# yui-mhcp/text_to_speech

Measured on AMD Instinct MI355X. Metric: audio samples/sec (22.05 kHz WaveGlow vocoding, fp32), higher is better.
Workload: dtype f32; 1 GPU; WaveGlow-only vocoding of precomputed 80x800 mel, batch 8 per GPU, fp32 (BASELINE.json configs[1]); batch_per_gpu=8, mel_frames=800, world_size=1, backend=single process, weights=seeded synthetic (rng 1234)

## Files before the change

### text_to_speech_amd/csrc/engine.h

```cpp
#pragma once
#include <hip/hip_runtime.h>
#include <stdint.h>

#include <cstdio>
#include <functional>
#include <map>
#include <string>
#include <tuple>
#include <vector>

#include "../../include/tts_hip.h"

#include "ttsw_host.h"
#include "wg_call.h"

struct DevBuf {
    void* p = nullptr;
    size_t bytes = 0;
    hipError_t ensure(size_t need) {
        if (need <= bytes) return hipSuccess;
        if (p) (void)hipFree(p);
        p = nullptr;
        bytes = 0;
        hipError_t e = hipMalloc(&p, need);
// ... 178 lines not shown
    std::map<std::string, HostTensor> host;
    WaveGlowDev wg;
    Tacotron2Dev taco;
    MelStftDev stft;
    AudioProcDev aproc;
    ResampleDev resamp;
    bool timing = false;
    std::vector<TimedLaunch> timed;
    std::vector<TimedLaunch> ev_pool;
    double time_sum_us[4] = {0, 0, 0, 0};
    int64_t time_cnt[4] = {0, 0, 0, 0};
};

int set_err(const tts_hip_engine* e, int code, const char* fmt, ...);

struct StreamScope {
    tts_hip_engine* e;
    hipStream_t saved;
    StreamScope(tts_hip_engine* eng, void* stream) : e(eng), saved(eng->stream) {
        if (stream) e->stream = (hipStream_t)stream;
    }
    ~StreamScope() { e->stream = saved; }
};

#define HIPCHK(e, call)                                                                                         \
    do {                                                                                                        \
        hipError_t _err = (call);                                                                               \
        if (_err != hipSuccess)                                                                                 \
            return set_err((e), TTS_HIP_EHIP, "%s:%d: %s -> %s", __FILE__, __LINE__, #call, hipGetErrorString(_err)); \
    } while (0)

int waveglow_build_wino(tts_hip_engine* e);
int waveglow_wino_begin(tts_hip_engine* e, const float* d_mel, int PR, int BT, int T, int form);
int waveglow_wino_layer(tts_hip_engine* e, const WgLayerDev& ly, int i, const float* x, float* acts_i, int PR, int BT, int T);
int waveglow_wino_layer0(tts_hip_engine* e, const WgLayerDev& ly, int h, const float* a0p, float* acts_0, int PR, int BT, int T);
void timing_begin(tts_hip_engine* e, int kind);
void timing_end(tts_hip_engine* e);
void timing_collect(tts_hip_engine* e);

int waveglow_finalize(tts_hip_engine* e);
int waveglow_run(tts_hip_engine* e, const float* d_mel, int B, int T, const float* d_z, float sigma, float* d_audio,
                 int precision, const int* d_lens = nullptr, const int* d_tail = nullptr, int n_tail = 0,
                 const int* d_flags = nullptr);
int waveglow_run_packed(tts_hip_engine* e, const float* d_mel, int B, int T, const float* d_z, float sigma, float* d_audio,
                        int precision, const int* d_info, int F, int n_gap);
void waveglow_free(tts_hip_engine* e);

int tacotron2_finalize(tts_hip_engine* e);
void tacotron2_free(tts_hip_engine* e);

int melstft_finalize(tts_hip_engine* e);
int melstft_run(tts_hip_engine* e, const float* d_audio, int B, int N, float* d_mel);
void melstft_free(tts_hip_engine* e);
void audioproc_free(tts_hip_engine* e);
void resample_free(tts_hip_engine* e);

int philox_fill(tts_hip_engine* e, float* out, long long n, uint64_t seed, uint64_t offset, int kind, hipStream_t st);
int philox_fill_rows(tts_hip_engine* e, float* out, int B, long long row_stride, const uint64_t* keys, const uint64_t* offsets,
                     const long long* counts, int kind, hipStream_t st);
const HostTensor* find_tensor(const tts_hip_engine* e, const std::string& name);
int upload(tts_hip_engine* e, const float* src, size_t n, float** dst, std::vector<void*>& allocs);
int dev_alloc(tts_hip_engine* e, size_t n_floats, float** dst, std::vector<void*>& allocs, bool zero);
```

### text_to_speech_amd/csrc/waveglow.hip

```cpp
#include "engine.h"
#include "gemm_f32.h"
#include "wg_plan.h"

#include <cmath>
#include <cstdlib>

using namespace ttsgemm;

namespace {

constexpr int C = 512;
constexpr int NCOND = 640;
constexpr int KCONV = 3 * C;
constexpr int KCONV0 = 3 * 16;
constexpr int KMEL = 4 * 80;
constexpr int NPH = 32;

__global__ void pack_bt_kernel(const float* __restrict__ src, int K, int src_ld, float* __restrict__ dst, int N,
                               long long ldb, int koff, int perm, int taps, int bk) {
    const long long idx = (long long)blockIdx.x * blockDim.x + threadIdx.x;
    if (idx >= (long long)N * K) return;
    const int n = (int)(idx / K), k = (int)(idx % K);
    int kd = k;
    if (taps > 1) {
// ... 919 lines not shown
    if (mask == MASK_FLAGS)
        hipLaunchKernelGGL(init_audio_kernel<MASK_FLAGS>, dim3(mb), dim3(256), 0, st, d_z, sigma, wg.audio.f(), PR, BT, d_flags, T);
    else if (mask == MASK_LENS)
        hipLaunchKernelGGL(init_audio_kernel<MASK_LENS>, dim3(mb), dim3(256), 0, st, d_z, sigma, wg.audio.f(), PR, BT, d_lens, T);
    else
        hipLaunchKernelGGL(init_audio_kernel<MASK_NONE>, dim3(mb), dim3(256), 0, st, d_z, sigma, wg.audio.f(), PR, BT, (const int*)nullptr, 1);
    if (precision != 0) {
        const long long n = (long long)BT * KMEL;
        hipLaunchKernelGGL(mel_window_kernel, dim3((unsigned)((n + 255) / 256)), dim3(256), 0, st, d_mel, mel16,
                           precision == 2 ? mel16 + n : (_Float16*)nullptr, BT, T);
    }
    HIPCHK(e, hipGetLastError());

    int zoff = 4;
    for (int k = 11; k >= 0; --k) {
        const WgFlowDev& fl = wg.flow[k];
        const int h = fl.n_half;
        {
            const long long n4 = M * (C / 4);
            const dim3 grid((unsigned)((n4 + 255) / 256));
            if (precision != 0)
                hipLaunchKernelGGL(wn_start_kernel<true>, grid, dim3(256), 0, st, wg.audio.f(), fl.start_w, fl.start_b,
                                   wg.x.f(), wg.a0p16.p, x16, M, h, precision == 2 ? 1 : 0);
            else
                hipLaunchKernelGGL(wn_start_kernel<false>, grid, dim3(256), 0, st, wg.audio.f(), fl.start_w, fl.start_b,
                                   wg.x.f(), wg.a0p.p, (_Float16*)nullptr, M, h);
            HIPCHK(e, hipGetLastError());
            if (int rc = zero_tail(true)) return rc;
        }
        for (int i = 0; i < 8; ++i) {
            const WgLayerDev& ly = fl.layer[i];
            const bool wino_layer = wino && i > 0;
            if (wino_layer) {
                if (int rc = waveglow_wino_layer(e, ly, i, wg.x.f(), call.acts_of(i), PR, BT, T)) return rc;
            } else if (wino) {
                if (int rc = waveglow_wino_layer0(e, ly, h, wg.a0p.f(), call.acts_of(0), PR, BT, T)) return rc;
            } else {
                const GemmArgs g = in_layer_args(call, ly, i);
                timing_begin(e, in_layer_timing_kind(precision, i));
                HIPCHK(e, (i == 0 ? kn.in0 : kn.in)(g, st));
                timing_end(e);
            }
            if (probe_wants_layer(wg, precision, k, i)) return probe_layer(e, call, i, wino_layer);
            if (i < 7) {
                const GemmArgs r = res_args(call, ly, i);
                timing_begin(e, 1);
                HIPCHK(e, kn.res(r, st));
                timing_end(e);
                if (int rc = zero_tail(false)) return rc;
            }
        }
        const bool early = (k % 4 == 0) && k > 0;
        float* dst = (k == 0) ? d_audio : wg.audio.f();
        const long long waves = (M + RPW - 1) / RPW;
        launch_end_fold(precision, mask, dim3((unsigned)((waves + 3) / 4)), st, (const void*)call.acts, plan.NP * M * C, fl.end_w,
                        fl.end_b, fl.inv, wg.audio.f(), dst, k == 0 ? 1 : 0, d_z, zoff, early ? 2 : 0, sigma, M, h, PR, BT,
                        precision == 2 ? M * C : 0ll, mask_info, mask == MASK_NONE ? 1 : T);
        HIPCHK(e, hipGetLastError());
        if (probe_wants_state(wg, k))
            return probe_state(e, plan, dst, k == 0 ? 1 : 0, 2 * h + (early ? 2 : 0));
        if (early) zoff += 2;
    }
    return TTS_HIP_OK;
}

int waveglow_run_packed(tts_hip_engine* e, const float* d_mel, int B, int T, const float* d_z, float sigma, float* d_audio,
                        int precision, const int* d_info, int F, int n_gap) {
// ... 24 lines not shown
```

### text_to_speech_amd/csrc/wn_wino.hip

```cpp
#include "engine.h"
#include "gemm_f32.h"
#include "wg_plan.h"

#include <algorithm>

using namespace ttsgemm;

namespace {
constexpr int C = 512;
constexpr int NPH = 32;
constexpr int KMEL = 320;
constexpr int KCONV = 3 * C;

__device__ __forceinline__ f32x4 x_at(const float* __restrict__ x, int ps, long long f, int df, int c, int PR, int BT, int T) {
    const f32x4 zero = {0.f, 0.f, 0.f, 0.f};
    if (f >= BT) return zero;
    const int carry = (ps >> 5) + df;
    const int t = (int)(f % T) + carry;
    if (t < 0 || t >= T) return zero;
    return *reinterpret_cast<const f32x4*>(x + ((long long)(ps & 31) * PR + f + carry) * C + c);
}


__device__ __forceinline__ int group_phase0(int gp, int d) { return (gp / d) * 4 * d + gp % d; }
// ... 159 lines not shown
    const int left = T - t0;
    tab[gr] = (long long)b * T < BT ? (b * T + t0) | (left < 4 ? left : 4) << 16 : 0;
}

struct WinoCondArgs {
    const float* Z;
    const int* rowtab;
    const float* W;
    const float* bias;
    float* cond;
    int rows;
    int PR, BT, T;
    const float* taps;
    const float* Wt;
    float* acts;
};

__global__ void wino_tap_operand_kernel(const float* __restrict__ a0p, float* __restrict__ taps, int h, int PR, int BT, int T) {
    const long long idx = (long long)blockIdx.x * blockDim.x + threadIdx.x;
    if (idx >= (long long)NPH * PR * 16) return;
    const int k = (int)(idx & 15);
    const long long m = idx >> 4;
    const int tap = wn_tap_of_col(k, h);
    const long long src = tap < 3 ? wn_tap_row((int)(m / PR), (int)(m % PR), tap - 1, PR, BT, T) : -1;
    taps[idx] = src >= 0 ? a0p[src * 16 + wn_tap_src_col(k, h)] : 0.f;
}
__global__ void wino_tap_weights_kernel(const float* __restrict__ in_Bt0, float* __restrict__ Wt, int h) {
    const int idx = blockIdx.x * blockDim.x + threadIdx.x;
    if (idx >= 2 * C * 16) return;
    const int k = idx & 15, tap = wn_tap_of_col(k, h);
    Wt[idx] = tap < 3 ? in_Bt0[(idx >> 4) * 48 + tap * 16 + wn_tap_src_col(k, h)] : 0.f;
}

template <int WR, int WC, int NBUF, bool L0>
__device__ __forceinline__ void wino_cond_body(const WinoCondArgs& g) {
    constexpr int NW = WR * WC, BM = WR * 32, BN = WC * 32;
    constexpr int NPA = BM / 16, NPB = BN / 16, PPW = (NPA + NPB) / NW;
    static_assert((NPA + NPB) % NW == 0 && PPW <= 4, "the pieces of a tile divide among the waves, one per MFMA of a half step");
    constexpr int STAGE = (BM + BN) * 16;
    constexpr int NKC = NMEL / 16, NT = NPT * NKC;
    typedef __attribute__((address_space(3))) void* lds_ptr_t;
    extern __shared__ __attribute__((aligned(16))) float smem[];
    const int tid = threadIdx.x, lane = tid & 63;
    const int wave = __builtin_amdgcn_readfirstlane(tid >> 6);
    const int wr = wave / WC, wc = wave % WC;
    const int li = lane & 31, lh = lane >> 5;

    constexpr int numNt = 2 * C / BN;
    const int numMt = g.rows / BM;
    const int bid = blockIdx.x, xcd = bid & 7, slot = bid >> 3;
    const int pair = (slot / numMt) * 8 + xcd, mt = slot % numMt;
    const int ph = pair / numNt, nt = pair % numNt;
    const int m0 = mt * BM, n0 = nt * BN;

    f32x16 acc[NPT];
#pragma unroll
    for (int p = 0; p < NPT; ++p)
#pragma unroll
        for (int r = 0; r < 16; ++r) acc[p][r] = 0.f;

    const int prow = lane >> 2, chunk = (lane & 3) ^ ((lane >> 4) & 3);
    unsigned vo0[PPW];
#pragma unroll
    for (int i = 0; i < PPW; ++i) {
        const int q = wave * PPW + i;
        const int row = (q < NPA ? q : q - NPA) * 16 + prow;
        vo0[i] = (unsigned)((row * NMEL + chunk * 4) * 4);
// ... 41 lines not shown
    asm volatile("s_waitcnt vmcnt(%0)" ::"n"(PPW * (NBUF - 1)) : "memory");
    __builtin_amdgcn_s_barrier();
    Frag f0, f1;
    read_frag(0, 0, f0);
    int buf = 0;
    static_for<NPT>([&](auto pc) {
        constexpr int P = decltype(pc)::value;
        for (int s = 0; s < NKC; ++s) {
            read_frag(buf, 1, f1);
            prepare();
#pragma unroll
            for (int kk = 0; kk < 4; ++kk) acc[P] = __builtin_amdgcn_mfma_f32_32x32x2f32(f0.a[kk], f0.b[kk], acc[P], 0, 0, 0);
            __builtin_amdgcn_sched_barrier(0);
            asm volatile("s_waitcnt vmcnt(%0) lgkmcnt(0)" ::"n"(PPW * (NBUF - 2)) : "memory");
            __builtin_amdgcn_s_barrier();
            const int bufn = buf == NBUF - 1 ? 0 : buf + 1;
            read_frag(bufn, 0, f0);
            __builtin_amdgcn_sched_barrier(0);
#pragma unroll
            for (int kk = 0; kk < 4; ++kk) {
                acc[P] = __builtin_amdgcn_mfma_f32_32x32x2f32(f1.a[kk], f1.b[kk], acc[P], 0, 0, 0);
                if (kk < PPW) {
                    issue_piece(kk, buf);
                    __builtin_amdgcn_sched_barrier(0);
                }
            }
            buf = bufn;
        }
    });
    asm volatile("s_waitcnt vmcnt(0)" ::: "memory");

    const float bv = g.bias[n0 + wc * 32 + li];
    const int* const rt = g.rowtab + m0 + wr * 32 + 4 * lh;
    if constexpr (!L0) {
        const __amdgpu_buffer_rsrc_t ro = make_rsrc_uniform(g.cond + (long long)ph * g.PR * (2 * C) + n0 + wc * 32);
#pragma unroll
        for (int r = 0; r < 16; ++r) {
            const int info = rt[(r & 3) + 8 * (r >> 2)];
            const unsigned voff = ((unsigned)(info & 0xffff) * (2 * C) + li) * 4u;
            const int nout = info >> 16;
            const float s12 = acc[1][r] + acc[2][r], d12 = acc[1][r] - acc[2][r];
            const float s34 = acc[3][r] + acc[4][r], d34 = acc[3][r] - acc[4][r];
            const float s56 = acc[5][r] + acc[6][r], d56 = acc[5][r] - acc[6][r];
            float y[4];
            y[0] = acc[0][r] + s12 + s34 + s56 + bv;
            y[1] = d12 + 2.f * d34 + 0.5f * d56 + bv;
            y[2] = s12 + 4.f * s34 + 0.25f * s56 + bv;
            y[3] = d12 + 8.f * d34 + 0.125f * d56 + bv;
#pragma unroll
            for (int j = 0; j < 4; ++j)
                __builtin_amdgcn_raw_buffer_store_b32(__builtin_bit_cast(unsigned, y[j]), ro, j < nout ? voff : OOB, j * (2 * C * 4), 0);
        }
    } else {
        static_assert(WC == 2, "waves (wr, 0) and (wr, 1) hold the tanh and the sigmoid half of the same 32 channels");
        const int arow = g.rowtab[m0 + wr * 32 + li];
        const __amdgpu_buffer_rsrc_t rta = make_rsrc_uniform(g.taps + (long long)ph * g.PR * 16);
        f32x4 ta[4][2], tb[2];
        auto load_taps = [&](int j) {
            const unsigned off = j < arow >> 16 ? ((unsigned)(arow & 0xffff) + j) * 64u + lh * 32u : OOB;
            ta[j][0] = buf_load4(rta, off);
            ta[j][1] = buf_load4(rta, off + 16u);
        };
        load_taps(0);
        load_taps(1);
        tb[0] = *reinterpret_cast<const f32x4*>(g.Wt + (n0 + wc * 32 + li) * 16 + lh * 8);
        tb[1] = *reinterpret_cast<const f32x4*>(g.Wt + (n0 + wc * 32 + li) * 16 + lh * 8 + 4);
#pragma unroll
        for (int r = 0; r < 16; ++r) {
            const float s12 = acc[1][r] + acc[2][r], d12 = acc[1][r] - acc[2][r];
            const float s34 = acc[3][r] + acc[4][r], d34 = acc[3][r] - acc[4][r];
            const float s56 = acc[5][r] + acc[6][r], d56 = acc[5][r] - acc[6][r];
            acc[0][r] = acc[0][r] + s12 + s34 + s56;
            acc[1][r] = d12 + 2.f * d34 + 0.5f * d56;
            acc[2][r] = s12 + 4.f * s34 + 0.25f * s56;
            acc[3][r] = d12 + 8.f * d34 + 0.125f * d56;
            if ((r & 3) == 3) __builtin_amdgcn_sched_barrier(0);
        }
        load_taps(2);
        load_taps(3);
#pragma unroll
        for (int j = 0; j < 4; ++j)
#pragma unroll
            for (int kk = 0; kk < 8; ++kk)
                acc[j] = __builtin_amdgcn_mfma_f32_32x32x2f32(ta[j][kk >> 2][kk & 3], tb[kk >> 2][kk & 3], acc[j], 0, 0, 0);
        float* const give = smem + wave * (32 * 64) + lane;
        const float* const take = smem + (wave ^ 1) * (32 * 64) + lane;
        __builtin_amdgcn_s_barrier();
        auto hand_over = [&](auto jc) {
            constexpr int JG = decltype(jc)::value;
#pragma unroll
            for (int jj = 0; jj < 2; ++jj)
#pragma unroll
                for (int r = 0; r < 16; ++r) give[(jj * 16 + r) * 64] = acc[JG + jj][r] + bv;
        };
        auto gate_store = [&](auto jc) {
            constexpr int JK = decltype(jc)::value;
            const __amdgpu_buffer_rsrc_t ro = make_rsrc_uniform(g.acts + (long long)ph * g.PR * C + (n0 >> 6) * 32);
#pragma unroll
            for (int r = 0; r < 16; ++r) {
                const int info = rt[(r & 3) + 8 * (r >> 2)];
                const unsigned voff = ((unsigned)(info & 0xffff) * C + li) * 4u;
                const int nout = info >> 16;
#pragma unroll
                for (int jj = 0; jj < 2; ++jj) {
                    const float mine = acc[JK + jj][r] + bv, other = take[(jj * 16 + r) * 64];
                    const float v = JK == 0 ? gate_tanh_sigmoid(mine, other) : gate_tanh_sigmoid(other, mine);
                    __builtin_amdgcn_raw_buffer_store_b32(__builtin_bit_cast(unsigned, v), ro, JK + jj < nout ? voff : OOB,
                                                          (JK + jj) * (C * 4), 0);
                }
            }
        };
        if (wc == 0) hand_over(std::integral_constant<int, 2>{});
        else hand_over(std::integral_constant<int, 0>{});
        asm volatile("s_waitcnt lgkmcnt(0)" ::: "memory");
        __builtin_amdgcn_s_barrier();
        if (wc == 0) gate_store(std::integral_constant<int, 0>{});
        else gate_store(std::integral_constant<int, 2>{});
    }
}

template <int WR, int WC, int NBUF, int OCC>
__global__ __launch_bounds__(WR * WC * 64, OCC) void wino_cond_kernel(const WinoCondArgs g) {
    wino_cond_body<WR, WC, NBUF, false>(g);
}
template <int WR, int WC, int NBUF, int OCC>
__global__ __launch_bounds__(WR * WC * 64, OCC) void wino_layer0_kernel(const WinoCondArgs g) {
    wino_cond_body<WR, WC, NBUF, true>(g);
}

template <int WR, int WC, int NBUF, int OCC, bool L0 = false>
hipError_t launch_wino_cond(const WinoCondArgs& a, hipStream_t st) {
    constexpr int BM = WR * 32, BN = WC * 32;
    const size_t lds = std::max((size_t)NBUF * (BM + BN) * 16, L0 ? (size_t)WR * WC * 32 * 64 : (size_t)0) * sizeof(float);
    if (a.rows % BM != 0) return hipErrorInvalidValue;
    auto kern = L0 ? wino_layer0_kernel<WR, WC, NBUF, OCC> : wino_cond_kernel<WR, WC, NBUF, OCC>;
    static PerDeviceOnce attr_set;
    if (hipError_t e = set_max_dyn_lds_once((const void*)kern, lds, attr_set); e != hipSuccess) return e;
    hipLaunchKernelGGL(kern, dim3((unsigned)(NPH * (2 * C / BN) * (a.rows / BM))), dim3(WR * WC * 64), lds, st, a);
    return hipGetLastError();
}

__device__ __forceinline__ unsigned group_out_pack(int kind, int gl, int sfr, int BT, int T) {
    if (kind == 0) return (unsigned)gl | 15u << 20;
    int b, t0;
    const bool ok = kind == 1 ? frame_group(gl, sfr, BT, T, b, t0) : mixed_group(gl, BT, T, b, t0);
    if (!ok) return 0u;
    const int left = T - t0;
    return (unsigned)(b * T + t0) | (unsigned)(left < 15 ? left : 15) << 20;
}
__device__ __forceinline__ long long group_out_base(int kind, int ph, int j, int d, int PR, unsigned& jstep) {
    if (kind == 0) {
        jstep = 0;
        return (long long)(group_phase0(ph, d) + j * d) * PR;
    }
    if (kind == 1) {
        jstep = (unsigned)(j * (d / NPH));
        return (long long)ph * PR + j * (d / NPH);
    }
    jstep = (unsigned)(j >> 1);
    return (long long)(ph + 16 * (j & 1)) * PR + (j >> 1);
}

__global__ void wino4_combine_kernel(const float* __restrict__ P, const float* __restrict__ cond, float* __restrict__ acts, int d,
                                     int PR, int BT, int T, long long Mq) {
    const long long idx = (long long)blockIdx.x * blockDim.x + threadIdx.x;
    if (idx >= Mq * (C / 4)) return;
    const long long mg = idx / (C / 4);
    const int ch = (int)(idx % (C / 4)) * 4;
// ... 72 lines not shown
                const float ct = ctv[rr], cs = csv[rr];
                float tv, sv;
                if constexpr (j == 0) {
                    tv = acc[0][0][r] + acc[1][0][r] + acc[2][0][r] + acc[3][0][r] + acc[4][0][r] + ct;
                    sv = acc[0][1][r] + acc[1][1][r] + acc[2][1][r] + acc[3][1][r] + acc[4][1][r] + cs;
                } else if constexpr (j == 1) {
                    tv = acc[1][0][r] - acc[2][0][r] + 2.f * (acc[3][0][r] - acc[4][0][r]) + ct;
                    sv = acc[1][1][r] - acc[2][1][r] + 2.f * (acc[3][1][r] - acc[4][1][r]) + cs;
                } else if constexpr (j == 2) {
                    tv = acc[1][0][r] + acc[2][0][r] + 4.f * (acc[3][0][r] + acc[4][0][r]) + ct;
                    sv = acc[1][1][r] + acc[2][1][r] + 4.f * (acc[3][1][r] + acc[4][1][r]) + cs;
                } else {
                    tv = acc[1][0][r] - acc[2][0][r] + 8.f * (acc[3][0][r] - acc[4][0][r]) + acc[5][0][r] + ct;
                    sv = acc[1][1][r] - acc[2][1][r] + 8.f * (acc[3][1][r] - acc[4][1][r]) + acc[5][1][r] + cs;
                }
                patch[((r & 3) + 8 * (r >> 2) + 4 * lh) * 36 + li] = gate_tanh_sigmoid(tv, sv);
            }
        }
        asm volatile("s_waitcnt lgkmcnt(0)" ::: "memory");
#pragma unroll
        for (int qq = 0; qq < 4; ++qq) {
            const f32x4 v = *reinterpret_cast<const f32x4*>(patch + (er + 8 * qq) * 36 + ec4);
            const unsigned srow = group_out_pack(kind, gl0 + er + 8 * qq, sfr, BT, T);
            if (jstep < srow >> 20) *reinterpret_cast<f32x4*>(acts + (jb + (srow & 0xfffffu)) * C + ch0) = v;
        }
        asm volatile("s_waitcnt lgkmcnt(0)" ::: "memory");
    });
}

__host__ __device__ constexpr int wino_stage_row(int k, int lane) { return 4 * k + (lane >> 4); }
__host__ __device__ constexpr int wino_stage_piece(int lane) { return (lane & 15) ^ (((lane >> 5) & 1) << 3); }
__host__ __device__ constexpr int wino_stage_at(int row, int col) { return row * 64 + (col ^ (((row >> 1) & 1) << 5)); }

__device__ __forceinline__ void wino_gate_store_dma(const f32x16 (&acc)[6][2], float* stage, const float* __restrict__ cond,
                                                    float* __restrict__ acts, int kind, int d, int ph, int gl0, int col0, int PR,
                                                    int BT, int T, int lane) {
    typedef __attribute__((address_space(3))) void* lds_ptr_t;
    constexpr int TILE = 32 * 64;
    const int li = lane & 31, lh = lane >> 5, er = lane >> 3, ec4 = (lane & 7) * 4;
    const int sfr = d / NPH;
    unsigned drow[8], srow[4];
#pragma unroll
    for (int k = 0; k < 8; ++k) {
        drow[k] = group_out_pack(kind, gl0 + wino_stage_row(k, lane), sfr, BT, T);
        __builtin_amdgcn_sched_barrier(0);
    }
#pragma unroll
    for (int qq = 0; qq < 4; ++qq) {
        srow[qq] = group_out_pack(kind, gl0 + er + 8 * qq, sfr, BT, T);
        __builtin_amdgcn_sched_barrier(0);
    }
    const unsigned dcol = (unsigned)wino_stage_piece(lane) * 16u;
    auto request = [&](auto jc) {
        constexpr int J = decltype(jc)::value;
        unsigned jstep;
        const long long jb = group_out_base(kind, ph, J, d, PR, jstep);
        const __amdgpu_buffer_rsrc_t rc = make_rsrc_uniform(cond + jb * (2 * C) + col0);
#pragma unroll
        for (int k = 0; k < 8; ++k) {
            const unsigned pk = drow[k];
            const unsigned voff = jstep < pk >> 20 ? (pk & 0xfffffu) * (2 * C * 4) + dcol : OOB;
            __builtin_amdgcn_raw_ptr_buffer_load_lds(rc, (lds_ptr_t)(stage + (J & 1) * TILE + k * 256), 16, voff, 0, 0, 0);
        }
    };
    request(std::integral_constant<int, 0>{});
    request(std::integral_constant<int, 1>{});
    static_for<4>([&](auto jc) {
        constexpr int j = decltype(jc)::value;
        unsigned jstep;
        const long long jb = group_out_base(kind, ph, j, d, PR, jstep);
        float* const mine = stage + (j & 1) * TILE + lh * (4 * 64) + li;
        asm volatile("s_waitcnt vmcnt(%0)" ::"n"(j == 0 ? 8 : j == 1 ? 12 : j == 2 ? 16 : 8) : "memory");
        constexpr int RB = j == 0 ? 8 : 16;
#pragma unroll
        for (int r0 = 0; r0 < 16; r0 += RB) {
            float ctv[RB], csv[RB];
#pragma unroll
            for (int rr = 0; rr < RB; ++rr) {
                const int r = r0 + rr, row = (r & 3) + 8 * (r >> 2);
                ctv[rr] = mine[wino_stage_at(row, 0)];
                csv[rr] = mine[wino_stage_at(row, 32)];
            }
            __builtin_amdgcn_sched_barrier(0);
#pragma unroll
            for (int rr = 0; rr < RB; ++rr) {
                const int r = r0 + rr;
                const float ct = ctv[rr], cs = csv[rr];
                float tv, sv;
                if constexpr (j == 0) {
                    tv = acc[0][0][r] + acc[1][0][r] + acc[2][0][r] + acc[3][0][r] + acc[4][0][r] + ct;
                    sv = acc[0][1][r] + acc[1][1][r] + acc[2][1][r] + acc[3][1][r] + acc[4][1][r] + cs;
                } else if constexpr (j == 1) {
                    tv = acc[1][0][r] - acc[2][0][r] + 2.f * (acc[3][0][r] - acc[4][0][r]) + ct;
                    sv = acc[1][1][r] - acc[2][1][r] + 2.f * (acc[3][1][r] - acc[4][1][r]) + cs;
                } else if constexpr (j == 2) {
                    tv = acc[1][0][r] + acc[2][0][r] + 4.f * (acc[3][0][r] + acc[4][0][r]) + ct;
                    sv = acc[1][1][r] + acc[2][1][r] + 4.f * (acc[3][1][r] + acc[4][1][r]) + cs;
                } else {
                    tv = acc[1][0][r] - acc[2][0][r] + 8.f * (acc[3][0][r] - acc[4][0][r]) + acc[5][0][r] + ct;
                    sv = acc[1][1][r] - acc[2][1][r] + 8.f * (acc[3][1][r] - acc[4][1][r]) + acc[5][1][r] + cs;
                }
                mine[wino_stage_at((r & 3) + 8 * (r >> 2), 0)] = gate_tanh_sigmoid(tv, sv);
            }
        }
        asm volatile("s_waitcnt lgkmcnt(0)" ::: "memory");
        f32x4 v[4];
#pragma unroll
        for (int qq = 0; qq < 4; ++qq)
            v[qq] = *reinterpret_cast<const f32x4*>(stage + (j & 1) * TILE + (er + 8 * qq) * 64 + (((er >> 1) & 1) << 5) + ec4);
        asm volatile("s_waitcnt lgkmcnt(0)" ::: "memory");
        if constexpr (j + 2 < 4) request(std::integral_constant<int, j + 2>{});
        const __amdgpu_buffer_rsrc_t ra = make_rsrc_uniform(acts + jb * C + (col0 >> 6) * 32);
#pragma unroll
        for (int qq = 0; qq < 4; ++qq) {
            const unsigned pk = srow[qq];
            const unsigned voff = jstep < pk >> 20 ? (pk & 0xfffffu) * (C * 4) + (unsigned)ec4 * 4u : OOB;
            __builtin_amdgcn_raw_buffer_store_b128(__builtin_bit_cast(u32x4, v[qq]), ra, voff, 0, 0);
        }
    });
}

struct WinoFusedArgs {
    const float* U;   long long uplane;
    const float* G;   long long gplane;
    const float* cond;
    float* acts;
    int Mq, phase_rows;
    int kind;
    int d, PR, BT, T;
};

template <int WR, int WC, int NBUF, int OCC>
__global__ __launch_bounds__(WR * WC * 64, OCC) void wino4_fused_kernel(const WinoFusedArgs g) {
    constexpr int NW = WR * WC, BM = WR * 32, BN = WC * 64;
    constexpr int NPA = BM / 16, NPB = BN / 16, PPW = (NPA + NPB) / NW;
    static_assert((NPA + NPB) % NW == 0, "the pieces of a tile divide among the waves");
    constexpr int STAGE = (BM + BN) * 16;
    static_assert(NBUF * STAGE >= NW * 32 * 36, "the epilogue's transpose patches fit the pipeline buffers");
    typedef __attribute__((address_space(3))) void* lds_ptr_t;
    extern __shared__ __attribute__((aligned(16))) float smem[];
    const int tid = threadIdx.x, lane = tid & 63;
    const int wave = __builtin_amdgcn_readfirstlane(tid >> 6);
    const int wr = wave / WC, wc = wave % WC;
    const int li = lane & 31, lh = lane >> 5;

    constexpr int numNt = 2 * C / BN;
    const int numMt = g.Mq / BM;
    const int bid = blockIdx.x, xcd = bid & 7, slot = bid >> 3;
    const int mt = (slot / numNt) * 8 + xcd, nt = slot % numNt;
    if (mt >= numMt) return;
    const int m0 = mt * BM, n0 = nt * BN;
// ... 84 lines not shown
                acc[P][0] = __builtin_amdgcn_mfma_f32_32x32x2f32(f1.a[kk], f1.b0[kk], acc[P][0], 0, 0, 0);
                acc[P][1] = __builtin_amdgcn_mfma_f32_32x32x2f32(f1.a[kk], f1.b1[kk], acc[P][1], 0, 0, 0);
                if (kk < PPW) {
                    issue_piece(kk, buf);
                    __builtin_amdgcn_sched_barrier(0);
                }
            }
            static_assert(PPW <= 4, "one DMA piece per MFMA pair of the second half");
            buf = bufn;
        }
    });
    asm volatile("s_waitcnt vmcnt(0)" ::: "memory");
    __builtin_amdgcn_s_barrier();

    wino_gate_store(acc, smem + wave * (32 * 36), g.cond, g.acts, g.kind, g.d, ph, fr0 + wr * 32, n0 + wc * 64, g.PR, g.BT, g.T, lane);
}

template <int WR, int WC, int NBUF, int OCC>
hipError_t launch_wino_fused(const WinoFusedArgs& a, hipStream_t st) {
    constexpr int BM = WR * 32, BN = WC * 64;
    const size_t lds = (size_t)NBUF * (BM + BN) * 16 * sizeof(float);
    if (a.Mq % BM != 0 || a.phase_rows % BM != 0 || a.Mq % a.phase_rows != 0) return hipErrorInvalidValue;
    auto kern = wino4_fused_kernel<WR, WC, NBUF, OCC>;
    static PerDeviceOnce attr_set;
    if (hipError_t e = set_max_dyn_lds_once((const void*)kern, lds, attr_set); e != hipSuccess) return e;
    const int numMt8 = (a.Mq / BM + 7) / 8 * 8;
    hipLaunchKernelGGL(kern, dim3(numMt8 * (2 * C / BN)), dim3(WR * WC * 64), lds, st, a);
    return hipGetLastError();
}

struct WinoFused2Args {
    const float* x;
    const float* G;   long long gplane;
    const float* cond;
    float* acts;
    int Mq, phase_rows, kind, d, PR, BT, T;
};

#ifdef TTS_WINO_STAMPS
__device__ unsigned long long g_wino_stamps[4 * 8192];
#define WINO_STAMP(i)                                                                               \
    do {                                                                                            \
        if (tid == 0 && bid < 8192) g_wino_stamps[4 * bid + (i)] = __builtin_amdgcn_s_memtime();    \
    } while (0)
#else
#define WINO_STAMP(i) do { } while (0)
#endif

__global__ __launch_bounds__(256, 2) void wino4_fused2_kernel(const WinoFused2Args g) {
    constexpr int BM = 64, BN = 128, NBUF = 3, NG = C / 16;
    constexpr int XT = BM * 16, XS = 6 * XT, BS = BN * 16;
    typedef __attribute__((address_space(3))) void* lds_ptr_t;
    extern __shared__ __attribute__((aligned(16))) float smem[];
    float* const xs = smem;
    float* const Bs = smem + 2 * XS;
    const int tid = threadIdx.x, lane = tid & 63;
    const int wave = __builtin_amdgcn_readfirstlane(tid >> 6);
    const int wr = wave >> 1, wc = wave & 1;
    const int li = lane & 31, lh = lane >> 5;

    constexpr int numNt = 2 * C / BN;
    const int numMt = g.Mq / BM;
    const int bid = blockIdx.x, xcd = bid & 7, slot = bid >> 3;
    const int mt = (slot / numNt) * 8 + xcd, nt = slot % numNt;
    if (mt >= numMt) return;
    const int m0 = mt * BM, n0 = nt * BN;
    const int ph = m0 / g.phase_rows, fr0 = m0 - ph * g.phase_rows;
#ifdef TTS_WINO_STAMPS
// ... 127 lines not shown
            __builtin_amdgcn_sched_barrier(0);
            f1.a = combine(pc, raw);
            read_b(buf, 1, f1);
            __builtin_amdgcn_sched_barrier(0);
            mfma2(pc, f0, 2);
            mfma2(pc, f0, 3);
            __builtin_amdgcn_sched_barrier(0);
            asm volatile("s_waitcnt vmcnt(3) lgkmcnt(0)" ::: "memory");
            __builtin_amdgcn_s_barrier();
            const int bufn = buf == NBUF - 1 ? 0 : buf + 1;
            read_x(std::integral_constant<int, PN>{}, P == 5 ? stage ^ 1 : stage, 0, raw);
            __builtin_amdgcn_sched_barrier(0);
            mfma2(pc, f1, 0);
            issue_x(std::integral_constant<int, XI>{}, grp + 1);
            __builtin_amdgcn_sched_barrier(0);
            mfma2(pc, f1, 1);
            __builtin_amdgcn_sched_barrier(0);
            f0.a = combine(std::integral_constant<int, PN>{}, raw);
            read_b(bufn, 0, f0);
            __builtin_amdgcn_sched_barrier(0);
            mfma2(pc, f1, 2);
            issue_b_taps(0, P3, grp + (P >= 3 ? 1 : 0), buf);
            __builtin_amdgcn_sched_barrier(0);
            mfma2(pc, f1, 3);
            issue_b_taps(1, P3, grp + (P >= 3 ? 1 : 0), buf);
            __builtin_amdgcn_sched_barrier(0);
            buf = bufn;
        });
    }
    asm volatile("s_waitcnt vmcnt(0)" ::: "memory");
    __builtin_amdgcn_s_barrier();
    WINO_STAMP(1);

    wino_gate_store_dma(acc, smem + wave * (2 * 32 * 64), g.cond, g.acts, g.kind, g.d, ph, fr0 + wr * 32, n0 + wc * 64, g.PR, g.BT, g.T,
                        lane);
    WINO_STAMP(2);
}

hipError_t launch_wino_fused2(const WinoFused2Args& a, hipStream_t st) {
    constexpr int BM = 64, BN = 128;
    const size_t lds = (size_t)(2 * 6 * BM * 16 + 3 * BN * 16) * sizeof(float);
    if (a.Mq % BM != 0 || a.phase_rows % BM != 0 || a.Mq % a.phase_rows != 0) return hipErrorInvalidValue;
    static PerDeviceOnce attr_set;
    if (hipError_t e = set_max_dyn_lds_once((const void*)wino4_fused2_kernel, lds, attr_set); e != hipSuccess) return e;
    const int numMt8 = (a.Mq / BM + 7) / 8 * 8;
    hipLaunchKernelGGL(wino4_fused2_kernel, dim3(numMt8 * (2 * C / BN)), dim3(256), lds, st, a);
    return hipGetLastError();
}

#ifdef TTS_WINO_STAMPS
}
extern "C" __attribute__((visibility("default"))) int tts_hip_debug_wino_stamps(unsigned long long* out, int n) {
    if (n < 0 || n > 8192 || hipDeviceSynchronize() != hipSuccess) return -1;
    return hipMemcpyFromSymbol(out, HIP_SYMBOL(g_wino_stamps), (size_t)n * 4 * sizeof(unsigned long long)) == hipSuccess ? 0 : -1;
}
namespace {
#endif

inline unsigned blocks_for(long long n) { return (unsigned)((n + 255) / 256); }
}

static inline int group_row_tile(int form) { return form == 2 ? 128 : 64; }
static inline int frame_group_rows(int BT, int T, int form) {
    const int g = group_row_tile(form);
    return ((BT / T) * frame_groups_per_utt(T) + g - 1) / g * g;
}
static inline int mixed_group_rows(int BT, int T, int form) {
    const int g = group_row_tile(form);
// ... 62 lines not shown
    if (wg.wino_cond.bytes != before) HIPCHK(e, hipMemsetAsync(wg.wino_cond.p, 0, wg.wino_cond.bytes, st));
    hipLaunchKernelGGL(wino_cond_mel_planes_kernel, dim3(blocks_for((long long)NPT * PRc * NMEL)), dim3(256), 0, st, d_mel,
                       wg.wino_mel.f(), PRc, BT, T);
    hipLaunchKernelGGL(wino_cond_rows_kernel, dim3(blocks_for(PRc)), dim3(256), 0, st, (int*)(wg.wino_mel.f() + (size_t)NPT * PRc * NMEL),
                       PRc, BT, T);
    HIPCHK(e, hipGetLastError());
    return TTS_HIP_OK;
}

static WinoCondArgs cond_args(WaveGlowDev& wg, const WgLayerDev& ly, int PR, int BT, int T) {
    WinoCondArgs c{};
    c.Z = wg.wino_mel.f();
    c.W = ly.wino_W;
    c.bias = ly.in_bias;
    c.cond = wg.wino_cond.f();
    c.rows = cond_group_rows(BT, T);
    c.rowtab = (const int*)(c.Z + (size_t)NPT * c.rows * NMEL);
    c.PR = PR;
    c.BT = BT;
    c.T = T;
    return c;
}

int waveglow_wino_layer0(tts_hip_engine* e, const WgLayerDev& ly, int h, const float* a0p, float* acts_0, int PR, int BT, int T) {
    WaveGlowDev& wg = e->wg;
    hipStream_t st = e->stream;
    WinoCondArgs c = cond_args(wg, ly, PR, BT, T);
    c.taps = wg.wino_taps.f();
    c.Wt = ly.wino_T;
    c.acts = acts_0;
    timing_begin(e, 3);
    hipLaunchKernelGGL(wino_tap_operand_kernel, dim3(blocks_for((long long)NPH * PR * 16)), dim3(256), 0, st, a0p, wg.wino_taps.f(), h,
                       PR, BT, T);
    HIPCHK(e, (launch_wino_cond<2, 2, 3, 3, true>(c, st)));
    timing_end(e);
    return TTS_HIP_OK;
}

int waveglow_wino_layer(tts_hip_engine* e, const WgLayerDev& ly, int i, const float* x, float* acts_i, int PR, int BT, int T) {
    WaveGlowDev& wg = e->wg;
    hipStream_t st = e->stream;
    const int d = 1 << i;
    float* U = wg.wino_U.f();
    float* P = wg.wino_P.f();
    const int PRq = frame_group_rows(BT, T, wg.form_mode), PRm = mixed_group_rows(BT, T, wg.form_mode);
    const bool phases = d <= 8, mixed = d == 16;
    const long long Mq = phases ? (long long)(NPH / 4) * PR : mixed ? (long long)16 * PRm : (long long)NPH * PRq;
    const WinoCondArgs c = cond_args(wg, ly, PR, BT, T);
    const bool no_prepass = wg.form_mode == 1;
    if (!no_prepass) hipLaunchKernelGGL(wino4_prepass_kernel, dim3(blocks_for(Mq * (C / 4))), dim3(256), 0, st, x, U, d, PR, BT, T, Mq);
    if (wg.form_mode != 2) {
        WinoFusedArgs a{};
        a.U = U;
        a.uplane = Mq * C;
        a.G = ly.wino_G;
        a.gplane = (long long)2 * C * C;
        a.cond = c.cond;
        a.acts = acts_i;
        a.Mq = (int)Mq;
        a.phase_rows = phases ? PR : mixed ? PRm : PRq;
        a.kind = phases ? 0 : mixed ? 2 : 1;
        a.d = d;
        a.PR = PR;
        a.BT = BT;
        a.T = T;
        if (no_prepass) {
            WinoFused2Args b{};
            b.x = x;
            b.G = a.G; b.gplane = a.gplane;
            b.cond = a.cond; b.acts = a.acts;
            b.Mq = a.Mq; b.phase_rows = a.phase_rows; b.kind = a.kind; b.d = a.d; b.PR = a.PR; b.BT = a.BT; b.T = a.T;
            timing_begin(e, 0);
            HIPCHK(e, (launch_wino_cond<2, 2, 3, 3>(c, st)));
            HIPCHK(e, launch_wino_fused2(b, st));
            timing_end(e);
            return TTS_HIP_OK;
        }
        timing_begin(e, 0);
        HIPCHK(e, (launch_wino_cond<2, 2, 3, 3>(c, st)));
        HIPCHK(e, (launch_wino_fused<2, 2, 3, 2>(a, st)));
        timing_end(e);
        return TTS_HIP_OK;
    }
    GemmArgs g{};
    g.M = (int)Mq;
    g.N = 2 * C;
    g.nphase = phases ? NPH / 4 : mixed ? 16 : NPH;
    g.phase_rows = phases ? PR : mixed ? PRm : PRq;
    g.frames = phases ? BT : mixed ? (BT / T) * mixed_groups_per_utt(T) : (BT / T) * frame_groups_per_utt(T);
    g.L = g.phase_rows;
    g.ldb = C;
    g.mode = EPI_LINEAR;
    g.act = ACT_NONE;
    g.split = 2 * C;
    g.ld0 = 2 * C;
    g.wide_epi = 1;
    g.nseg = 1;
    g.seg[0] = ASeg{U, C, 0, C, C, SEG_ROWS_Z, 0, Mq, 0};
    g.Bt = ly.wino_G;
    g.strideBz = (long long)2 * C * C;
    g.out0 = P;
    g.strideOutZ = Mq * 2 * C;
    timing_begin(e, 0);
    HIPCHK(e, (launch_wino_cond<2, 2, 3, 3>(c, st)));
    HIPCHK(e, phases && PR % 256 == 0 ? gemm_wn_wino(g, 6, st) : gemm_wn_wino_128(g, 6, st));
    timing_end(e);
    hipLaunchKernelGGL(wino4_combine_kernel, dim3(blocks_for(Mq * (C / 4))), dim3(256), 0, st, P, c.cond, acts_i, d, PR, BT, T, Mq);
// ... 4 lines not shown
```

Measured before the change: 4.605 million audio samples/s.

## Move WaveGlow gate epilogue from fused conv kernel into conditioning GEMM

```diff
diff --git a/text_to_speech_amd/csrc/engine.h b/text_to_speech_amd/csrc/engine.h
--- a/text_to_speech_amd/csrc/engine.h
+++ b/text_to_speech_amd/csrc/engine.h
@@ -234,7 +234,8 @@
 
 int waveglow_build_wino(tts_hip_engine* e);
 int waveglow_wino_begin(tts_hip_engine* e, const float* d_mel, int PR, int BT, int T, int form);
-int waveglow_wino_layer(tts_hip_engine* e, const WgLayerDev& ly, int i, const float* x, float* acts_i, int PR, int BT, int T);
+int waveglow_wino_layer(tts_hip_engine* e, const WgLayerDev& ly, int i, const float* x, float* acts_i, int PR, int BT, int T,
+                        bool plane_only);
 int waveglow_wino_layer0(tts_hip_engine* e, const WgLayerDev& ly, int h, const float* a0p, float* acts_0, int PR, int BT, int T);
 void timing_begin(tts_hip_engine* e, int kind);
 void timing_end(tts_hip_engine* e);
diff --git a/text_to_speech_amd/csrc/waveglow.hip b/text_to_speech_amd/csrc/waveglow.hip
--- a/text_to_speech_amd/csrc/waveglow.hip
+++ b/text_to_speech_amd/csrc/waveglow.hip
@@ -975,7 +975,8 @@
             const WgLayerDev& ly = fl.layer[i];
             const bool wino_layer = wino && i > 0;
             if (wino_layer) {
-                if (int rc = waveglow_wino_layer(e, ly, i, wg.x.f(), call.acts_of(i), PR, BT, T)) return rc;
+                const bool plane_only = probe_wants_layer(wg, precision, k, i) && wg.probe_what == 2;
+                if (int rc = waveglow_wino_layer(e, ly, i, wg.x.f(), call.acts_of(i), PR, BT, T, plane_only)) return rc;
             } else if (wino) {
                 if (int rc = waveglow_wino_layer0(e, ly, h, wg.a0p.f(), call.acts_of(0), PR, BT, T)) return rc;
             } else {
diff --git a/text_to_speech_amd/csrc/wn_wino.hip b/text_to_speech_amd/csrc/wn_wino.hip
--- a/text_to_speech_amd/csrc/wn_wino.hip
+++ b/text_to_speech_amd/csrc/wn_wino.hip
@@ -215,7 +215,8 @@
     Wt[idx] = tap < 3 ? in_Bt0[(idx >> 4) * 48 + tap * 16 + wn_tap_src_col(k, h)] : 0.f;
 }
 
-template <int WR, int WC, int NBUF, bool L0>
+constexpr int CEPI_PLANE = 0, CEPI_L0 = 1, CEPI_GATE = 2;
+template <int WR, int WC, int NBUF, int EPI>
 __device__ __forceinline__ void wino_cond_body(const WinoCondArgs& g) {
     constexpr int NW = WR * WC, BM = WR * 32, BN = WC * 32;
     constexpr int NPA = BM / 16, NPB = BN / 16, PPW = (NPA + NPB) / NW;
@@ -323,7 +324,7 @@
 
     const float bv = g.bias[n0 + wc * 32 + li];
     const int* const rt = g.rowtab + m0 + wr * 32 + 4 * lh;
-    if constexpr (!L0) {
+    if constexpr (EPI == CEPI_PLANE) {
         const __amdgpu_buffer_rsrc_t ro = make_rsrc_uniform(g.cond + (long long)ph * g.PR * (2 * C) + n0 + wc * 32);
 #pragma unroll
         for (int r = 0; r < 16; ++r) {
@@ -342,7 +343,7 @@
             for (int j = 0; j < 4; ++j)
                 __builtin_amdgcn_raw_buffer_store_b32(__builtin_bit_cast(unsigned, y[j]), ro, j < nout ? voff : OOB, j * (2 * C * 4), 0);
         }
-    } else {
+    } else if constexpr (EPI == CEPI_L0) {
         static_assert(WC == 2, "waves (wr, 0) and (wr, 1) hold the tanh and the sigmoid half of the same 32 channels");
         const int arow = g.rowtab[m0 + wr * 32 + li];
         const __amdgpu_buffer_rsrc_t rta = make_rsrc_uniform(g.taps + (long long)ph * g.PR * 16);
@@ -374,6 +375,51 @@
 #pragma unroll
             for (int kk = 0; kk < 8; ++kk)
                 acc[j] = __builtin_amdgcn_mfma_f32_32x32x2f32(ta[j][kk >> 2][kk & 3], tb[kk >> 2][kk & 3], acc[j], 0, 0, 0);
+    } else {
+        static_assert(WC == 2, "waves (wr, 0) and (wr, 1) hold the tanh and the sigmoid half of the same 32 channels");
+        const __amdgpu_buffer_rsrc_t rp = make_rsrc_uniform(g.cond + (long long)ph * g.PR * (2 * C) + n0 + wc * 32);
+        f32x16 pa, pb;
+        auto load_pre = [&](int j, f32x16& p) {
+#pragma unroll
+            for (int r = 0; r < 16; ++r) {
+                const int info = rt[(r & 3) + 8 * (r >> 2)];
+                const unsigned voff = j < info >> 16 ? ((unsigned)(info & 0xffff) * (2 * C) + li) * 4u : OOB;
+                p[r] = __builtin_bit_cast(float, __builtin_amdgcn_raw_buffer_load_b32(rp, voff, j * (2 * C * 4), 0));
+            }
+            __builtin_amdgcn_sched_barrier(0);
+        };
+        auto add_pre = [&](auto jc, const f32x16& p) {
+            constexpr int J = decltype(jc)::value;
+#pragma unroll
+            for (int r = 0; r < 16; ++r) acc[J][r] = acc[J][r] + bv + p[r];
+            asm volatile("" : "+v"(acc[J]));
+            __builtin_amdgcn_sched_barrier(0);
+        };
+        load_pre(0, pa);
+        asm volatile("" ::: "memory");
+#pragma unroll
+        for (int r = 0; r < 16; ++r) {
+            const float s12 = acc[1][r] + acc[2][r], d12 = acc[1][r] - acc[2][r];
+            const float s34 = acc[3][r] + acc[4][r], d34 = acc[3][r] - acc[4][r];
+            const float s56 = acc[5][r] + acc[6][r], d56 = acc[5][r] - acc[6][r];
+            acc[0][r] = acc[0][r] + s12 + s34 + s56;
+            acc[1][r] = d12 + 2.f * d34 + 0.5f * d56;
+            acc[2][r] = s12 + 4.f * s34 + 0.25f * s56;
+            acc[3][r] = d12 + 8.f * d34 + 0.125f * d56;
+            if ((r & 3) == 3) __builtin_amdgcn_sched_barrier(0);
+        }
+        asm volatile("" : "+v"(acc[0]), "+v"(acc[1]), "+v"(acc[2]), "+v"(acc[3]));
+        __builtin_amdgcn_sched_barrier(0);
+        load_pre(1, pb);
+        add_pre(std::integral_constant<int, 0>{}, pa);
+        load_pre(2, pa);
+        add_pre(std::integral_constant<int, 1>{}, pb);
+        load_pre(3, pb);
+        add_pre(std::integral_constant<int, 2>{}, pa);
+        add_pre(std::integral_constant<int, 3>{}, pb);
+    }
+    if constexpr (EPI != CEPI_PLANE) {
+        auto biased = [&](float v) { return EPI == CEPI_L0 ? v + bv : v; };
         float* const give = smem + wave * (32 * 64) + lane;
         const float* const take = smem + (wave ^ 1) * (32 * 64) + lane;
         __builtin_amdgcn_s_barrier();
@@ -382,7 +428,7 @@
 #pragma unroll
             for (int jj = 0; jj < 2; ++jj)
 #pragma unroll
-                for (int r = 0; r < 16; ++r) give[(jj * 16 + r) * 64] = acc[JG + jj][r] + bv;
+                for (int r = 0; r < 16; ++r) give[(jj * 16 + r) * 64] = biased(acc[JG + jj][r]);
         };
         auto gate_store = [&](auto jc) {
             constexpr int JK = decltype(jc)::value;
@@ -394,7 +440,7 @@
                 const int nout = info >> 16;
 #pragma unroll
                 for (int jj = 0; jj < 2; ++jj) {
-                    const float mine = acc[JK + jj][r] + bv, other = take[(jj * 16 + r) * 64];
+                    const float mine = biased(acc[JK + jj][r]), other = take[(jj * 16 + r) * 64];
                     const float v = JK == 0 ? gate_tanh_sigmoid(mine, other) : gate_tanh_sigmoid(other, mine);
                     __builtin_amdgcn_raw_buffer_store_b32(__builtin_bit_cast(unsigned, v), ro, JK + jj < nout ? voff : OOB,
                                                           (JK + jj) * (C * 4), 0);
@@ -412,19 +458,25 @@
 
 template <int WR, int WC, int NBUF, int OCC>
 __global__ __launch_bounds__(WR * WC * 64, OCC) void wino_cond_kernel(const WinoCondArgs g) {
-    wino_cond_body<WR, WC, NBUF, false>(g);
+    wino_cond_body<WR, WC, NBUF, CEPI_PLANE>(g);
 }
 template <int WR, int WC, int NBUF, int OCC>
 __global__ __launch_bounds__(WR * WC * 64, OCC) void wino_layer0_kernel(const WinoCondArgs g) {
-    wino_cond_body<WR, WC, NBUF, true>(g);
-}
-
-template <int WR, int WC, int NBUF, int OCC, bool L0 = false>
+    wino_cond_body<WR, WC, NBUF, CEPI_L0>(g);
+}
+template <int WR, int WC, int NBUF, int OCC>
+__global__ __launch_bounds__(WR * WC * 64, OCC) void wino_cond_gate_kernel(const WinoCondArgs g) {
+    wino_cond_body<WR, WC, NBUF, CEPI_GATE>(g);
+}
+
+template <int WR, int WC, int NBUF, int OCC, int EPI = CEPI_PLANE>
 hipError_t launch_wino_cond(const WinoCondArgs& a, hipStream_t st) {
     constexpr int BM = WR * 32, BN = WC * 32;
-    const size_t lds = std::max((size_t)NBUF * (BM + BN) * 16, L0 ? (size_t)WR * WC * 32 * 64 : (size_t)0) * sizeof(float);
+    const size_t lds = std::max((size_t)NBUF * (BM + BN) * 16, EPI != CEPI_PLANE ? (size_t)WR * WC * 32 * 64 : (size_t)0) * sizeof(float);
     if (a.rows % BM != 0) return hipErrorInvalidValue;
-    auto kern = L0 ? wino_layer0_kernel<WR, WC, NBUF, OCC> : wino_cond_kernel<WR, WC, NBUF, OCC>;
+    auto kern = EPI == CEPI_L0     ? wino_layer0_kernel<WR, WC, NBUF, OCC>
+                : EPI == CEPI_GATE ? wino_cond_gate_kernel<WR, WC, NBUF, OCC>
+                                  : wino_cond_kernel<WR, WC, NBUF, OCC>;
     static PerDeviceOnce attr_set;
     if (hipError_t e = set_max_dyn_lds_once((const void*)kern, lds, attr_set); e != hipSuccess) return e;
     hipLaunchKernelGGL(kern, dim3((unsigned)(NPH * (2 * C / BN) * (a.rows / BM))), dim3(WR * WC * 64), lds, st, a);
@@ -563,91 +615,61 @@
 __host__ __device__ constexpr int wino_stage_piece(int lane) { return (lane & 15) ^ (((lane >> 5) & 1) << 3); }
 __host__ __device__ constexpr int wino_stage_at(int row, int col) { return row * 64 + (col ^ (((row >> 1) & 1) << 5)); }
 
-__device__ __forceinline__ void wino_gate_store_dma(const f32x16 (&acc)[6][2], float* stage, const float* __restrict__ cond,
-                                                    float* __restrict__ acts, int kind, int d, int ph, int gl0, int col0, int PR,
-                                                    int BT, int T, int lane) {
-    typedef __attribute__((address_space(3))) void* lds_ptr_t;
+__device__ __forceinline__ void wino_pre_store(const f32x16 (&acc)[6][2], float* stage, float* __restrict__ pre, int kind, int d,
+                                               int ph, int gl0, int col0, int PR, int BT, int T, int lane) {
     constexpr int TILE = 32 * 64;
-    const int li = lane & 31, lh = lane >> 5, er = lane >> 3, ec4 = (lane & 7) * 4;
+    const int li = lane & 31, lh = lane >> 5;
     const int sfr = d / NPH;
-    unsigned drow[8], srow[4];
+    unsigned srow[8];
 #pragma unroll
     for (int k = 0; k < 8; ++k) {
-        drow[k] = group_out_pack(kind, gl0 + wino_stage_row(k, lane), sfr, BT, T);
+        srow[k] = group_out_pack(kind, gl0 + wino_stage_row(k, lane), sfr, BT, T);
         __builtin_amdgcn_sched_barrier(0);
     }
-#pragma unroll
-    for (int qq = 0; qq < 4; ++qq) {
-        srow[qq] = group_out_pack(kind, gl0 + er + 8 * qq, sfr, BT, T);
-        __builtin_amdgcn_sched_barrier(0);
-    }
     const unsigned dcol = (unsigned)wino_stage_piece(lane) * 16u;
-    auto request = [&](auto jc) {
-        constexpr int J = decltype(jc)::value;
-        unsigned jstep;
-        const long long jb = group_out_base(kind, ph, J, d, PR, jstep);
-        const __amdgpu_buffer_rsrc_t rc = make_rsrc_uniform(cond + jb * (2 * C) + col0);
-#pragma unroll
-        for (int k = 0; k < 8; ++k) {
-            const unsigned pk = drow[k];
-            const unsigned voff = jstep < pk >> 20 ? (pk & 0xfffffu) * (2 * C * 4) + dcol : OOB;
-            __builtin_amdgcn_raw_ptr_buffer_load_lds(rc, (lds_ptr_t)(stage + (J & 1) * TILE + k * 256), 16, voff, 0, 0, 0);
-        }
-    };
-    request(std::integral_constant<int, 0>{});
-    request(std::integral_constant<int, 1>{});
-    static_for<4>([&](auto jc) {
-        constexpr int j = decltype(jc)::value;
-        unsigned jstep;
-        const long long jb = group_out_base(kind, ph, j, d, PR, jstep);
-        float* const mine = stage + (j & 1) * TILE + lh * (4 * 64) + li;
-        asm volatile("s_waitcnt vmcnt(%0)" ::"n"(j == 0 ? 8 : j == 1 ? 12 : j == 2 ? 16 : 8) : "memory");
-        constexpr int RB = j == 0 ? 8 : 16;
-#pragma unroll
-        for (int r0 = 0; r0 < 16; r0 += RB) {
-            float ctv[RB], csv[RB];
-#pragma unroll
-            for (int rr = 0; rr < RB; ++rr) {
-                const int r = r0 + rr, row = (r & 3) + 8 * (r >> 2);
-                ctv[rr] = mine[wino_stage_at(row, 0)];
-                csv[rr] = mine[wino_stage_at(row, 32)];
+    float* const mine = stage + lh * (4 * 64) + li;
+    static_for<2>([&](auto pc) {
+        constexpr int JA = decltype(pc)::value == 0 ? 1 : 0, JB = JA + 2;
+#pragma unroll
+        for (int r = 0; r < 16; ++r) {
+            float ta, sa, tb, sb;
+            if constexpr (JA == 1) {
+                ta = acc[1][0][r] - acc[2][0][r] + 2.f * (acc[3][0][r] - acc[4][0][r]);
+                sa = acc[1][1][r] - acc[2][1][r] + 2.f * (acc[3][1][r] - acc[4][1][r]);
+                tb = acc[1][0][r] - acc[2][0][r] + 8.f * (acc[3][0][r] - acc[4][0][r]) + acc[5][0][r];
+                sb = acc[1][1][r] - acc[2][1][r] + 8.f * (acc[3][1][r] - acc[4][1][r]) + acc[5][1][r];
+            } else {
+                ta = acc[0][0][r] + acc[1][0][r] + acc[2][0][r] + acc[3][0][r] + acc[4][0][r];
+                sa = acc[0][1][r] + acc[1][1][r] + acc[2][1][r] + acc[3][1][r] + acc[4][1][r];
+                tb = acc[1][0][r] + acc[2][0][r] + 4.f * (acc[3][0][r] + acc[4][0][r]);
+                sb = acc[1][1][r] + acc[2][1][r] + 4.f * (acc[3][1][r] + acc[4][1][r]);
             }
-            __builtin_amdgcn_sched_barrier(0);
-#pragma unroll
-            for (int rr = 0; rr < RB; ++rr) {
-                const int r = r0 + rr;
-                const float ct = ctv[rr], cs = csv[rr];
-                float tv, sv;
-                if constexpr (j == 0) {
-                    tv = acc[0][0][r] + acc[1][0][r] + acc[2][0][r] + acc[3][0][r] + acc[4][0][r] + ct;
-                    sv = acc[0][1][r] + acc[1][1][r] + acc[2][1][r] + acc[3][1][r] + acc[4][1][r] + cs;
-                } else if constexpr (j == 1) {
-                    tv = acc[1][0][r] - acc[2][0][r] + 2.f * (acc[3][0][r] - acc[4][0][r]) + ct;
-                    sv = acc[1][1][r] - acc[2][1][r] + 2.f * (acc[3][1][r] - acc[4][1][r]) + cs;
-                } else if constexpr (j == 2) {
-                    tv = acc[1][0][r] + acc[2][0][r] + 4.f * (acc[3][0][r] + acc[4][0][r]) + ct;
-                    sv = acc[1][1][r] + acc[2][1][r] + 4.f * (acc[3][1][r] + acc[4][1][r]) + cs;
-                } else {
-                    tv = acc[1][0][r] - acc[2][0][r] + 8.f * (acc[3][0][r] - acc[4][0][r]) + acc[5][0][r] + ct;
-                    sv = acc[1][1][r] - acc[2][1][r] + 8.f * (acc[3][1][r] - acc[4][1][r]) + acc[5][1][r] + cs;
+            const int row = (r & 3) + 8 * (r >> 2);
+            mine[wino_stage_at(row, 0)] = ta;
+            mine[wino_stage_at(row, 32)] = sa;
+            mine[TILE + wino_stage_at(row, 0)] = tb;
+            mine[TILE + wino_stage_at(row, 32)] = sb;
+        }
+        asm volatile("s_waitcnt lgkmcnt(0)" ::: "memory");
+        static_for<2>([&](auto sc) {
+            constexpr int S = decltype(sc)::value, j = S == 0 ? JA : JB;
+            unsigned jstep;
+            const long long jb = group_out_base(kind, ph, j, d, PR, jstep);
+            const __amdgpu_buffer_rsrc_t rp = make_rsrc_uniform(pre + jb * (2 * C) + col0);
+#pragma unroll
+            for (int k0 = 0; k0 < 8; k0 += 4) {
+                f32x4 v[4];
+#pragma unroll
+                for (int kk = 0; kk < 4; ++kk) v[kk] = *reinterpret_cast<const f32x4*>(stage + S * TILE + (k0 + kk) * 256 + lane * 4);
+#pragma unroll
+                for (int kk = 0; kk < 4; ++kk) {
+                    const unsigned pk = srow[k0 + kk];
+                    const unsigned voff = jstep < pk >> 20 ? (pk & 0xfffffu) * (2 * C * 4) + dcol : OOB;
+                    __builtin_amdgcn_raw_buffer_store_b128(__builtin_bit_cast(u32x4, v[kk]), rp, voff, 0, 0);
                 }
-                mine[wino_stage_at((r & 3) + 8 * (r >> 2), 0)] = gate_tanh_sigmoid(tv, sv);
             }
-        }
-        asm volatile("s_waitcnt lgkmcnt(0)" ::: "memory");
-        f32x4 v[4];
-#pragma unroll
-        for (int qq = 0; qq < 4; ++qq)
-            v[qq] = *reinterpret_cast<const f32x4*>(stage + (j & 1) * TILE + (er + 8 * qq) * 64 + (((er >> 1) & 1) << 5) + ec4);
-        asm volatile("s_waitcnt lgkmcnt(0)" ::: "memory");
-        if constexpr (j + 2 < 4) request(std::integral_constant<int, j + 2>{});
-        const __amdgpu_buffer_rsrc_t ra = make_rsrc_uniform(acts + jb * C + (col0 >> 6) * 32);
-#pragma unroll
-        for (int qq = 0; qq < 4; ++qq) {
-            const unsigned pk = srow[qq];
-            const unsigned voff = jstep < pk >> 20 ? (pk & 0xfffffu) * (C * 4) + (unsigned)ec4 * 4u : OOB;
-            __builtin_amdgcn_raw_buffer_store_b128(__builtin_bit_cast(u32x4, v[qq]), ra, voff, 0, 0);
-        }
+        });
+        asm volatile("" ::: "memory");
     });
 }
 
@@ -798,8 +820,7 @@
 struct WinoFused2Args {
     const float* x;
     const float* G;   long long gplane;
-    const float* cond;
-    float* acts;
+    float* pre;
     int Mq, phase_rows, kind, d, PR, BT, T;
 };
 
@@ -993,8 +1014,7 @@
     __builtin_amdgcn_s_barrier();
     WINO_STAMP(1);
 
-    wino_gate_store_dma(acc, smem + wave * (2 * 32 * 64), g.cond, g.acts, g.kind, g.d, ph, fr0 + wr * 32, n0 + wc * 64, g.PR, g.BT, g.T,
-                        lane);
+    wino_pre_store(acc, smem + wave * (2 * 32 * 64), g.pre, g.kind, g.d, ph, fr0 + wr * 32, n0 + wc * 64, g.PR, g.BT, g.T, lane);
     WINO_STAMP(2);
 }
 
@@ -1123,12 +1143,13 @@
     timing_begin(e, 3);
     hipLaunchKernelGGL(wino_tap_operand_kernel, dim3(blocks_for((long long)NPH * PR * 16)), dim3(256), 0, st, a0p, wg.wino_taps.f(), h,
                        PR, BT, T);
-    HIPCHK(e, (launch_wino_cond<2, 2, 3, 3, true>(c, st)));
+    HIPCHK(e, (launch_wino_cond<2, 2, 3, 3, CEPI_L0>(c, st)));
     timing_end(e);
     return TTS_HIP_OK;
 }
 
-int waveglow_wino_layer(tts_hip_engine* e, const WgLayerDev& ly, int i, const float* x, float* acts_i, int PR, int BT, int T) {
+int waveglow_wino_layer(tts_hip_engine* e, const WgLayerDev& ly, int i, const float* x, float* acts_i, int PR, int BT, int T,
+                        bool plane_only) {
     WaveGlowDev& wg = e->wg;
     hipStream_t st = e->stream;
     const int d = 1 << i;
@@ -1139,6 +1160,10 @@
     const long long Mq = phases ? (long long)(NPH / 4) * PR : mixed ? (long long)16 * PRm : (long long)NPH * PRq;
     const WinoCondArgs c = cond_args(wg, ly, PR, BT, T);
     const bool no_prepass = wg.form_mode == 1;
+    if (plane_only) {
+        HIPCHK(e, (launch_wino_cond<2, 2, 3, 3>(c, st)));
+        return TTS_HIP_OK;
+    }
     if (!no_prepass) hipLaunchKernelGGL(wino4_prepass_kernel, dim3(blocks_for(Mq * (C / 4))), dim3(256), 0, st, x, U, d, PR, BT, T, Mq);
     if (wg.form_mode != 2) {
         WinoFusedArgs a{};
@@ -1159,11 +1184,13 @@
             WinoFused2Args b{};
             b.x = x;
             b.G = a.G; b.gplane = a.gplane;
-            b.cond = a.cond; b.acts = a.acts;
+            b.pre = wg.wino_cond.f();
             b.Mq = a.Mq; b.phase_rows = a.phase_rows; b.kind = a.kind; b.d = a.d; b.PR = a.PR; b.BT = a.BT; b.T = a.T;
+            WinoCondArgs cg = c;
+            cg.acts = acts_i;
             timing_begin(e, 0);
-            HIPCHK(e, (launch_wino_cond<2, 2, 3, 3>(c, st)));
             HIPCHK(e, launch_wino_fused2(b, st));
+            HIPCHK(e, (launch_wino_cond<2, 2, 3, 3, CEPI_GATE>(cg, st)));
             timing_end(e);
             return TTS_HIP_OK;
         }
```

Result: no change. 4.640 million audio samples/s (median of 6 runs) (+0.7%).
